# peleiden/rl-rubiks

Hardware: NVIDIA B200
Metric: cube_moves_per_sec (higher is better)
Workload: dtype u8

## Files before the change

### include/rubiks_b200.h

```cpp
#ifndef RUBIKS_B200_H
#define RUBIKS_B200_H

#include <stdint.h>

#ifdef __cplusplus
extern "C" {
#endif

#define RB_OK              0
#define RB_ERR_BAD_ARG     1
#define RB_ERR_CUDA        2
#define RB_ERR_RANGE       3
#define RB_ERR_CAPACITY    4

#define RB_REP_2024        0
#define RB_REP_686         1

#define RB_REWARD_PAPER      0
#define RB_REWARD_LAPANFIX   1
#define RB_REWARD_SCHULTZFIX 2
#define RB_REWARD_REWARD0    3

typedef void* rb_stream_t;

int         rb_version(void);
const char* rb_last_error(void);
int64_t     rb_launch_count(void);

int rb_get_delta_maps(int8_t* delta);
int rb_get_lut2024(uint8_t* lut);
int rb_get_perm686(uint8_t* perm);
int rb_get_macro_table(uint32_t* rows);
int rb_get_macro3_table(uint32_t* rows);
int rb_get_macro3_dedup(uint32_t* elems, uint32_t* remap);
int rb_get_stickers686(uint8_t* corner_home, uint8_t* corner_dst, uint8_t* edge_home, uint8_t* edge_dst);
int rb_get_solved(int rep, int8_t* state);

int rb_multi_rotate(int rep, const int8_t* states, const uint8_t* faces, const uint8_t* dirs,
                    int8_t* out, int64_t n, rb_stream_t stream);
int rb_multi_is_solved(int rep, const int8_t* states, uint8_t* flags, int64_t n, rb_stream_t stream);
int rb_as_oh(int rep, const int8_t* states, float* oh, int64_t n, rb_stream_t stream);
int rb_as_correct_686(const float* oh, float* out, int64_t n, rb_stream_t stream);
int rb_expand12(int rep, const int8_t* states, int8_t* children, float* children_oh,
                uint8_t* solved, int64_t n, rb_stream_t stream);
int rb_check_range(int rep, const int8_t* states, int64_t n_states, const uint8_t* faces,
                   const uint8_t* dirs, int64_t n_actions, int32_t* scratch_dev, rb_stream_t stream);

int rb_scramble(int rep, const uint8_t* actions, int64_t stride_cube, int64_t stride_move,
                const int8_t* start, int8_t* out, int64_t n, int32_t depth, rb_stream_t stream);
int rb_sequence_scramble(int rep, const uint8_t* faces, const uint8_t* dirs, int32_t games, int32_t depth,
                         int32_t with_solved, int8_t* states, float* oh, uint8_t* solved, rb_stream_t stream);

int rb_scramble_seeded(int rep, uint64_t seed, uint64_t first_cube, const int8_t* start, int8_t* out, int64_t n,
                       int32_t depth, rb_stream_t stream);
int rb_seeded_actions(uint64_t seed, uint64_t first_cube, uint8_t* actions, int64_t n, int32_t depth, rb_stream_t stream);
int rb_unpack_actions(const uint8_t* packed, uint8_t* actions, int64_t n, int32_t depth, rb_stream_t stream);

int rb_as686(const int8_t* states2024, int8_t* states686, int64_t n, rb_stream_t stream);
int rb_as2024(const int8_t* states686, int8_t* states2024, uint8_t* ok, int64_t n, rb_stream_t stream);

int rb_adi_generate(int rep, const uint8_t* faces, const uint8_t* dirs, int32_t games, int32_t depth,
                    int32_t with_solved, int8_t* states, float* oh_states, int8_t* children,
                    float* children_oh, uint8_t* solved_states, uint8_t* solved_children, rb_stream_t stream);

int rb_as_oh_bf16(int rep, const int8_t* states, uint16_t* oh, int64_t n, rb_stream_t stream);
int rb_expand12_bf16(int rep, const int8_t* states, int8_t* children, uint16_t* children_oh,
                     uint8_t* solved, int64_t n, rb_stream_t stream);
int rb_sequence_scramble_bf16(int rep, const uint8_t* faces, const uint8_t* dirs, int32_t games, int32_t depth,
                              int32_t with_solved, int8_t* states, uint16_t* oh, uint8_t* solved, rb_stream_t stream);
int rb_adi_generate_bf16(int rep, const uint8_t* faces, const uint8_t* dirs, int32_t games, int32_t depth,
                         int32_t with_solved, int8_t* states, uint16_t* oh_states, int8_t* children,
                         uint16_t* children_oh, uint8_t* solved_states, uint8_t* solved_children, rb_stream_t stream);
int rb_adi_targets(const float* values, const uint8_t* solved_children, const uint8_t* solved_states,
                   int64_t n, int32_t depth, int32_t reward_method, int64_t* policy, float* value,
                   rb_stream_t stream);
int rb_adi_targets_weights(const float* values, const uint8_t* solved_children, const uint8_t* solved_states,
                           int32_t games, int32_t depth, int32_t reward_method, double alpha, double ws,
                           int64_t* policy, float* value, float* loss_weights, rb_stream_t stream);
double rb_adi_weight_sum(int32_t games, int32_t depth);
int rb_adi_loss_weights(float* out, int32_t games, int32_t depth, double alpha, double ws, rb_stream_t stream);

int64_t rb_hashset_bytes(int64_t capacity);
int rb_hashset_clear(void* table, int64_t capacity, rb_stream_t stream);
int rb_hashset_rehash(void* src, int64_t src_capacity, void* dst, int64_t dst_capacity, rb_stream_t stream);
int64_t rb_hashset_scratch_bytes(int64_t n);
int rb_hashset_insert_unique(int rep, void* table, int64_t capacity, const int8_t* states, int64_t n,
                             int32_t* count_dev, uint8_t* seen, uint8_t* first, int32_t* index,
// ... 52 lines not shown
```

### rl_rubiks_b200/_native.py

```python
from __future__ import annotations

import ctypes as C
import os

_HERE = os.path.dirname(os.path.abspath(__file__))
LIB_PATH = os.environ.get("RB_LIB_PATH") or os.path.join(_HERE, "librubiks_b200.so")

RB_OK, RB_ERR_BAD_ARG, RB_ERR_CUDA, RB_ERR_RANGE, RB_ERR_CAPACITY = 0, 1, 2, 3, 4
REP_2024, REP_686 = 0, 1
REWARD_METHODS = {"paper": 0, "lapanfix": 1, "schultzfix": 2, "reward0": 3}

if not os.path.exists(LIB_PATH):
	raise ImportError(
		f"{LIB_PATH} is missing: build it with `python -c 'import __graft_entry__ as g; g.build()'` "
		"(nvcc, sm_100a).  rl_rubiks_b200 has no CPU fallback.")

lib = C.CDLL(LIB_PATH)

_p, _i32, _i64, _f64 = C.c_void_p, C.c_int32, C.c_int64, C.c_double

SIGNATURES = {
	"rb_version": (C.c_int, []),
	"rb_last_error": (C.c_char_p, []),
	"rb_launch_count": (_i64, []),
	"rb_get_delta_maps": (C.c_int, [_p]),
	"rb_get_lut2024": (C.c_int, [_p]),
	"rb_get_perm686": (C.c_int, [_p]),
	"rb_get_macro_table": (C.c_int, [_p]),
	"rb_get_macro3_table": (C.c_int, [_p]),
	"rb_get_macro3_dedup": (C.c_int, [_p, _p]),
	"rb_get_stickers686": (C.c_int, [_p, _p, _p, _p]),
	"rb_get_solved": (C.c_int, [C.c_int, _p]),
	"rb_multi_rotate": (C.c_int, [C.c_int, _p, _p, _p, _p, _i64, _p]),
	"rb_multi_is_solved": (C.c_int, [C.c_int, _p, _p, _i64, _p]),
	"rb_as_oh": (C.c_int, [C.c_int, _p, _p, _i64, _p]),
	"rb_as_correct_686": (C.c_int, [_p, _p, _i64, _p]),
	"rb_expand12": (C.c_int, [C.c_int, _p, _p, _p, _p, _i64, _p]),
	"rb_check_range": (C.c_int, [C.c_int, _p, _i64, _p, _p, _i64, _p, _p]),
	"rb_scramble": (C.c_int, [C.c_int, _p, _i64, _i64, _p, _p, _i64, _i32, _p]),
	"rb_sequence_scramble": (C.c_int, [C.c_int, _p, _p, _i32, _i32, _i32, _p, _p, _p, _p]),
	"rb_adi_generate": (C.c_int, [C.c_int, _p, _p, _i32, _i32, _i32, _p, _p, _p, _p, _p, _p, _p]),
	"rb_as_oh_bf16": (C.c_int, [C.c_int, _p, _p, _i64, _p]),
	"rb_expand12_bf16": (C.c_int, [C.c_int, _p, _p, _p, _p, _i64, _p]),
	"rb_sequence_scramble_bf16": (C.c_int, [C.c_int, _p, _p, _i32, _i32, _i32, _p, _p, _p, _p]),
	"rb_adi_generate_bf16": (C.c_int, [C.c_int, _p, _p, _i32, _i32, _i32, _p, _p, _p, _p, _p, _p, _p]),
	"rb_adi_targets": (C.c_int, [_p, _p, _p, _i64, _i32, _i32, _p, _p, _p]),
	"rb_adi_targets_weights": (C.c_int, [_p, _p, _p, _i32, _i32, _i32, _f64, _f64, _p, _p, _p, _p]),
	"rb_adi_weight_sum": (_f64, [_i32, _i32]),
	"rb_adi_loss_weights": (C.c_int, [_p, _i32, _i32, _f64, _f64, _p]),
	"rb_hashset_bytes": (_i64, [_i64]),
	"rb_hashset_clear": (C.c_int, [_p, _i64, _p]),
	"rb_hashset_rehash": (C.c_int, [_p, _i64, _p, _i64, _p]),
	"rb_hashset_scratch_bytes": (_i64, [_i64]),
	"rb_hashset_insert_unique": (C.c_int, [C.c_int, _p, _i64, _p, _i64, _p, _p, _p, _p, _p, _p]),
	"rb_hashset_lookup": (C.c_int, [C.c_int, _p, _i64, _p, _i64, _p, _p, _p]),
	"rb_frontier_expand": (C.c_int, [C.c_int, _p, _i64, _p, _i64, _p, _p, _p, _p, _p, _p, _p, _p, _p, _p, _p]),
	"rb_frontier_expand_dev": (C.c_int, [C.c_int, _p, _i64, _p, _i64, _p, _p, _p, _p, _p, _p, _p, _p, _p]),
	"rb_frontier_expand_chain": (C.c_int, [C.c_int, _p, _i64, _p, _p, _i64, _i32, _p, _p, _p, _p]),
	"rb_frontier_scratch_bytes": (_i64, [C.c_int, _i64]),
	"rb_astar_scratch_bytes": (_i64, [_i32, _i32]),
	"rb_astar_init": (C.c_int, [_p, _p, _p]),
	"rb_astar_expand": (C.c_int, [_p, _i64, _p, _p, _p, _p, _p, _p]),
	"rb_astar_commit": (C.c_int, [_p, _p, _f64, _p, _p, _p, _p]),
	"rb_as686": (C.c_int, [_p, _p, _i64, _p]),
	"rb_as2024": (C.c_int, [_p, _p, _p, _i64, _p]),
	"rb_scramble_seeded": (C.c_int, [C.c_int, C.c_uint64, C.c_uint64, _p, _p, _i64, _i32, _p]),
	"rb_seeded_actions": (C.c_int, [C.c_uint64, C.c_uint64, _p, _i64, _i32, _p]),
	"rb_unpack_actions": (C.c_int, [_p, _p, _i64, _i32, _p]),
	"rbh_scramble": (C.c_int, [C.c_int, _p, _p, _i64, _i32]),
	"rbh_scramble_packed": (C.c_int, [C.c_int, _p, _p, _i64, _i32]),
	"rbh_scramble_seeded": (C.c_int, [C.c_int, C.c_uint64, C.c_uint64, _p, _i64, _i32]),
	"rbh_multi_rotate": (C.c_int, [C.c_int, _p, _p, _p, _p, _i64]),
	"rbh_host_alloc": (_p, [_i64, C.c_int]),
	"rbh_host_free": (C.c_int, [_p, _i64]),
	"rbh_release": (C.c_int, []),
}

for _name, (_res, _args) in SIGNATURES.items():
	_fn = getattr(lib, _name)
	_fn.restype, _fn.argtypes = _res, _args


class AStarView(C.Structure):
# ... 32 lines not shown
```

### rl_rubiks_b200/csrc/rb_scramble_macro.cuh

```cuda
#pragma once
#include "rb_common.cuh"
#include "rb_tables.cuh"
#include <cuda.h>
#include <array>
#include <map>

namespace rbs {

constexpr int kA = 13;
constexpr int kRows = kA * kA;
constexpr int kRowWords = 5;
constexpr int kDevRows = 256;
constexpr int kP1Bytes = kDevRows * 8 * 16;
constexpr int kP2Bytes = kDevRows * 32 * 4;
constexpr int kTableBytes = kP1Bytes + kP2Bytes;
constexpr int kMaxThreads = 1024;
constexpr int kSmemBudget = 227 * 1024;
constexpr int kReduceEvery = 10;

__device__ __align__(16) uint32_t g_macro[kRows * kRowWords + 3];
__device__ __align__(16) uint32_t g_macro3[12 * 12 * 12 * kRowWords + 3];
__device__ __align__(16) uint32_t g_macro_tail_inv[13 * 13 * kRowWords + 3];

struct Elem {
	uint8_t csrc[8], ctw[8], esrc[12], efl[12];
};

static inline bool neg_chirality(int pos) { return pos == 0 || pos == 2 || pos == 5 || pos == 7; }
static inline int twist_of(int pos, int ori) { return neg_chirality(pos) ? (3 - ori) % 3 : ori; }

static bool single(const rbt::Tables& t, int a, Elem& e) {
	for (int q = 0; q < 8; ++q) { e.csrc[q] = (uint8_t)q; e.ctw[q] = 0; }
	for (int q = 0; q < 12; ++q) { e.esrc[q] = (uint8_t)q; e.efl[q] = 0; }
	if (a == 12) return true;
	for (int p = 0; p < 8; ++p) {
		int delta = -1, dst = -1;
		for (int o = 0; o < 3; ++o) {
			const int v = t.lut[a][0][3 * p + o], p2 = v / 3, o2 = v % 3;
			const int d = (twist_of(p2, o2) - twist_of(p, o) + 3) % 3;
			if (o == 0) { delta = d; dst = p2; }
			else if (d != delta || p2 != dst) return false;
		}
		e.csrc[dst] = (uint8_t)p;
		e.ctw[dst] = (uint8_t)delta;
	}
	for (int p = 0; p < 12; ++p) {
		const int v0 = t.lut[a][1][2 * p], v1 = t.lut[a][1][2 * p + 1];
		if (v0 / 2 != v1 / 2 || ((v0 % 2) ^ 0) != ((v1 % 2) ^ 1)) return false;
		e.esrc[v0 / 2] = (uint8_t)p;
		e.efl[v0 / 2] = (uint8_t)(v0 % 2);
	}
	return true;
}

static void compose(const Elem& x, const Elem& y, Elem& r) {
	for (int q = 0; q < 8; ++q) {
		r.csrc[q] = x.csrc[y.csrc[q]];
		r.ctw[q] = (uint8_t)((x.ctw[y.csrc[q]] + y.ctw[q]) % 3);
	}
	for (int q = 0; q < 12; ++q) {
		r.esrc[q] = x.esrc[y.esrc[q]];
		r.efl[q] = (uint8_t)(x.efl[y.esrc[q]] ^ y.efl[q]);
	}
}

static void encode(const Elem& e, uint32_t* row) {
	uint32_t sc = 0, tf = 0;
	for (int q = 0; q < 8; ++q) sc |= (uint32_t)e.csrc[q] << (4 * q);
	for (int i = 0; i < 4; ++i) tf |= ((uint32_t)e.ctw[i] | ((uint32_t)e.ctw[4 + i] << 2)) << (8 * i);
	row[0] = sc;
	for (int d = 0; d < 3; ++d) {
		uint32_t sa = 0, sb = 0;
		for (int i = 0; i < 4; ++i) {
			const int s = e.esrc[4 * d + i];
			sa |= (uint32_t)(s < 8 ? s : 0) << (4 * i);
			sb |= (uint32_t)(s < 8 ? i : 4 + (s - 8)) << (4 * i);
			tf |= (uint32_t)e.efl[4 * d + i] << (8 * i + 4 + d);
		}
		row[1 + d] = sa | (sb << 16);
	}
	row[4] = tf;
}

constexpr int kRows3 = 12 * 12 * 12;

constexpr int kElems3 = 1080;
constexpr int kRepDedup = 8;
constexpr int kSingle3 = 15 + 12 * 15 + 144 * 15 + 1;
constexpr int kRemap3 = kSingle3 + 16;
constexpr int kElemBytes3 = kElems3 * kRepDedup * 16;
constexpr int kImageBytes3 = kElemBytes3 + kRemap3 * 8;
__device__ __align__(16) uint32_t g_macro3_image[kImageBytes3 / 4];

struct Host {
	uint32_t rows[kRows * kRowWords + 3];
	uint32_t rows3[kRows3 * kRowWords + 3];
	uint32_t rows3_inv[kRows3 * kRowWords + 3];
	uint32_t rows_inv[kRows * kRowWords + 3];
	uint32_t elems3[kElems3 * 4];
	uint32_t remap3[kRemap3 * 2];
	uint32_t image3[kImageBytes3 / 4];
	bool ok;
};

static const Host& host() {
	static Host h;
	static std::once_flag once;
	std::call_once(once, [] {
		memset(&h, 0, sizeof(h));
		const rbt::Tables& t = rbt::host();
		Elem s[kA];
		h.ok = true;
		for (int a = 0; a < kA; ++a) h.ok = single(t, a, s[a]) && h.ok;
		for (int a1 = 0; a1 < kA; ++a1)
			for (int a0 = 0; a0 < kA; ++a0) {
				Elem x;
				compose(s[a0], s[a1], x);
				encode(x, h.rows + (a0 + kA * a1) * kRowWords);
				if (a0 < 12 && a1 < 12)
					for (int a2 = 0; a2 < 12; ++a2) {
						Elem y;
						compose(x, s[a2], y);
						encode(y, h.rows3 + (a0 + 12 * a1 + 144 * a2) * kRowWords);
					}
			}
		auto inv = [](int a) { return a < 12 ? a ^ 1 : a; };
		for (int i = 0; i < kRows3; ++i) {
			const int j = inv(i % 12) + 12 * inv(i / 12 % 12) + 144 * inv(i / 144);
			memcpy(h.rows3_inv + i * kRowWords, h.rows3 + j * kRowWords, sizeof(uint32_t) * kRowWords);
		}
		for (int i = 0; i < kRows; ++i) {
			const int j = inv(i % kA) + kA * inv(i / kA);
			memcpy(h.rows_inv + i * kRowWords, h.rows + j * kRowWords, sizeof(uint32_t) * kRowWords);
		}

		std::map<std::array<uint32_t, 4>, uint32_t> elem;
		auto element_of = [&](const uint32_t* r) {
			const std::array<uint32_t, 4> key{r[0], r[1], r[2], r[3]};
			auto it = elem.find(key);
			if (it != elem.end()) return it->second;
			const uint32_t e = (uint32_t)elem.size();
			if (e < (uint32_t)kElems3) memcpy(h.elems3 + 4 * e, r, 16);
			elem.emplace(key, e);
			return e;
		};
		for (int i = 0; i < kRows3; ++i) {
			const uint32_t* r = h.rows3_inv + i * kRowWords;
			h.remap3[2 * i] = r[4];
			h.remap3[2 * i + 1] = element_of(r);
		}
		for (int a = 0; a < 12; ++a) {
			uint32_t r[kRowWords];
			encode(s[a ^ 1], r);
			h.remap3[2 * (kSingle3 + a)] = r[4];
			h.remap3[2 * (kSingle3 + a) + 1] = element_of(r);
		}
		h.ok = h.ok && elem.size() == (size_t)kElems3;
		auto same = [&](int i, const uint32_t* r) {
			const uint32_t e = h.remap3[2 * i + 1];
			return e < (uint32_t)kElems3 && memcmp(h.elems3 + 4 * e, r, 16) == 0 && h.remap3[2 * i] == r[4];
		};
		for (int i = 0; i < kRows3; ++i) h.ok = h.ok && same(i, h.rows3_inv + i * kRowWords);
		for (int a = 0; a < 12; ++a) h.ok = h.ok && same(kSingle3 + a, h.rows_inv + (a + kA * 12) * kRowWords);
		for (int e = 0; e < kElems3; ++e)
			for (int c = 0; c < kRepDedup; ++c) memcpy(h.image3 + (e * kRepDedup + c) * 4, h.elems3 + 4 * e, 16);
		memcpy(h.image3 + kElemBytes3 / 4, h.remap3, sizeof(h.remap3));
	});
	return h;
}

__device__ __forceinline__ uint32_t smem_u32(const void* p) { return (uint32_t)__cvta_generic_to_shared(p); }

__device__ __forceinline__ void mbar_init(uint64_t* bar, uint32_t count) {
	asm volatile("mbarrier.init.shared::cta.b64 [%0], %1;" ::"r"(smem_u32(bar)), "r"(count) : "memory");
}
__device__ __forceinline__ void mbar_expect_tx(uint64_t* bar, uint32_t bytes) {
	asm volatile("mbarrier.arrive.expect_tx.shared::cta.b64 _, [%0], %1;" ::"r"(smem_u32(bar)), "r"(bytes) : "memory");
}
__device__ __forceinline__ void mbar_wait(uint64_t* bar, uint32_t parity) {
	asm volatile(
		"{\n\t"
		".reg .pred p;\n\t"
		"WAIT_%=:\n\t"
		"mbarrier.try_wait.parity.shared::cta.b64 p, [%0], %1;\n\t"
		"@p bra DONE_%=;\n\t"
		"bra WAIT_%=;\n\t"
		"DONE_%=:\n\t"
		"}" ::"r"(smem_u32(bar)), "r"(parity) : "memory");
}
__device__ __forceinline__ void bulk_g2s(void* dst_smem, const void* src_gmem, uint32_t bytes, uint64_t* bar) {
	asm volatile("cp.async.bulk.shared::cluster.global.mbarrier::complete_tx::bytes [%0], [%1], %2, [%3];" ::"r"(smem_u32(dst_smem)),
	             "l"(src_gmem), "r"(bytes), "r"(smem_u32(bar))
	             : "memory");
}

__device__ __forceinline__ void tma_2d_g2s(void* dst_smem, const CUtensorMap* map, int32_t x, int32_t y, uint64_t* bar) {
	asm volatile("cp.async.bulk.tensor.2d.shared::cluster.global.tile.mbarrier::complete_tx::bytes [%0], [%1, {%2, %3}], [%4];" ::"r"(smem_u32(dst_smem)),
	             "l"(map), "r"(x), "r"(y), "r"(smem_u32(bar))
	             : "memory");
}

struct Slots {
	uint32_t C0, C1, E0, E1, E2;
};

__device__ __forceinline__ uint32_t prmt(uint32_t a, uint32_t b, uint32_t sel) {
	uint32_t r;
	asm("prmt.b32 %0, %1, %2, %3;" : "=r"(r) : "r"(a), "r"(b), "r"(sel));
	return r;
}
template <int k>
__device__ __forceinline__ uint32_t shr_fma(uint32_t x) {
	uint32_t r;
	asm("mul.hi.u32 %0, %1, %2;" : "=r"(r) : "r"(x), "r"(1u << (32 - k)));
	return r;
}

__device__ __forceinline__ uint32_t shr16(uint32_t x) {
	uint32_t r;
// ... 120 lines not shown
				for (; m < depth; m += 2) {
					const uint32_t a0 = row[m], a1 = m + 1 < depth ? row[m + 1] : 12u;
					apply_at(table, row_offset((a0 & 15u) + 13u * (a1 & 15u), lane_off), d2, s);
				}
			}
			store_state(row, s);
		}
		__syncwarp();
		{
			uint8_t* dst = reinterpret_cast<uint8_t*>(out) + chunk * 32 * out_pitch;
			if (kWordAligned && (reinterpret_cast<uintptr_t>(out) & 3u) == 0) {
				for (int i = lane; i < cnt * 5; i += 32) {
					const int c = i / 5, k = i - 5 * c;
					*reinterpret_cast<uint32_t*>(dst + c * out_pitch + 4 * k) = *reinterpret_cast<const uint32_t*>(buf + c * depth + 4 * k);
				}
			} else {
				for (int i = lane; i < cnt * 20; i += 32) {
					const int c = i / 20, k = i - 20 * c;
					dst[c * out_pitch + k] = buf[c * depth + k];
				}
			}
		}
		asm volatile("fence.proxy.async.shared::cta;" ::: "memory");
		__syncwarp();
		if (lane == 0 && chunk + stride < n_chunks) issue(chunk + stride);
	}
}

constexpr int kRep1 = 4;
constexpr int kIdxMax3 = 15 + 12 * 15 + 144 * 15;
constexpr int kP1Bytes3 = kRows3 * kRep1 * 16;
constexpr int kP2Rows3 = 2368;
constexpr int kP2Bytes3 = kP2Rows3 * 4;
constexpr int kTailBytes = kDevRows * 32;
constexpr int kTableBytes3 = kP1Bytes3 + kP2Bytes3 + kTailBytes;
constexpr int kMinSmem3 = (kIdxMax3 + 1) * kRep1 * 16 + 128;

__device__ __forceinline__ uint32_t mad_u32(uint32_t a, uint32_t b, uint32_t c) {
	uint32_t o;
	asm("mad.lo.u32 %0, %1, %2, %3;" : "=r"(o) : "r"(a), "r"(b), "r"(c));
	return o;
}

__device__ __forceinline__ uint4 lds128(uint32_t a) {
	uint4 v;
	asm("ld.shared.v4.u32 {%0, %1, %2, %3}, [%4];" : "=r"(v.x), "=r"(v.y), "=r"(v.z), "=r"(v.w) : "r"(a));
	return v;
}
__device__ __forceinline__ uint32_t lds32(uint32_t a) {
	uint32_t v;
	asm("ld.shared.u32 %0, [%1];" : "=r"(v) : "r"(a));
	return v;
}
__device__ __forceinline__ uint2 lds64(uint32_t a) {
	uint2 v;
	asm("ld.shared.v2.u32 {%0, %1}, [%2];" : "=r"(v.x), "=r"(v.y) : "r"(a));
	return v;
}

__device__ __forceinline__ void stage_table3(uint8_t* table) {
	for (int i = threadIdx.x; i < kP2Rows3 * kRep1; i += blockDim.x) {
		const int row = i / kRep1, c = i % kRep1;
		if (row < kRows3) {
			const uint32_t* r = g_macro3 + row * kRowWords;
			*reinterpret_cast<uint4*>(table + (row * kRep1 + c) * 16) = make_uint4(r[0], r[1], r[2], r[3]);
			if (c == 0) *reinterpret_cast<uint32_t*>(table + kP1Bytes3 + row * 4) = r[4];
		} else if (c == 0) {
			*reinterpret_cast<uint32_t*>(table + kP1Bytes3 + row * 4) = 0u;
		}
	}
	uint8_t* tail = table + kP1Bytes3 + kP2Bytes3;
	for (int i = threadIdx.x; i < kDevRows; i += blockDim.x) {
		const uint32_t* r = g_macro_tail_inv + (i < kRows ? i : kRows - 1) * kRowWords;
		*reinterpret_cast<uint4*>(tail + i * 32) = make_uint4(r[0], r[1], r[2], r[3]);
		*reinterpret_cast<uint32_t*>(tail + i * 32 + 16) = r[4];
	}
}

__device__ __forceinline__ void fold(Slots& s) { s.C0 = fold_twists(s.C0); s.C1 = fold_twists(s.C1); }

template <bool kDedup>
struct Rows3 {
	uint32_t off1, off2, tail, p1_stride, p2_stride;

	__device__ __forceinline__ Rows3(const uint8_t* table, uint32_t lane, uint32_t p1, uint32_t p2)
		: off1(smem_u32(table) + (lane & ((kDedup ? kRepDedup : kRep1) - 1)) * 16u),
		  off2(smem_u32(table) + (kDedup ? (uint32_t)kElemBytes3 : (uint32_t)kP1Bytes3)),
		  tail(smem_u32(table + kP1Bytes3 + kP2Bytes3)), p1_stride(p1), p2_stride(p2) {}

	__device__ __forceinline__ void apply3(Slots& s, uint32_t r) const {
		if (kDedup) {
			const uint2 e = lds64(mad_u32(r, p2_stride, off2));
			apply_row(lds128(mad_u32(e.y, p1_stride, off1)), e.x, s);
		} else {
			const uint32_t o1 = mad_u32(r, 16u * kRep1, off1), o2 = mad_u32(r, p2_stride, off2);
			apply_row(lds128(o1), lds32(o2), s);
		}
	}
	__device__ __forceinline__ void apply1(Slots& s, uint32_t a) const { apply3(s, (uint32_t)kSingle3 + a); }
	__device__ __forceinline__ void apply_tail(Slots& s, uint32_t idx2) const {
		const uint32_t r = tail + idx2 * 32u;
		apply_row(lds128(r), lds32(r + 16u), s);
	}
	__device__ __forceinline__ void apply_words(Slots& s, uint32_t w0, uint32_t w1, uint32_t w2) const {
		w0 &= 0x0f0f0f0fu; w1 &= 0x0f0f0f0fu; w2 &= 0x0f0f0f0fu;
		apply3(s, __dp4a(w2, 0x010C9000u, 0u));
		apply3(s, __dp4a(w2, 0x00000001u, __dp4a(w1, 0x0C900000u, 0u)));
		apply3(s, __dp4a(w1, 0x0000010Cu, __dp4a(w0, 0x90000000u, 0u)));
		apply3(s, __dp4a(w0, 0x00010C90u, 0u));
	}
	__device__ __forceinline__ void rem8(Slots& s, uint32_t wa, uint32_t wb) const {
		wa &= 0x0f0f0f0fu; wb &= 0x0f0f0f0fu;
		apply3(s, __dp4a(wb, 0x010C9000u, 0u));
		apply3(s, __dp4a(wb, 0x00000001u, __dp4a(wa, 0x0C900000u, 0u)));
		if (kDedup) { apply1(s, (wa >> 8) & 0xffu); apply1(s, wa & 0xffu); }
		else apply_tail(s, __dp4a(wa, 0x0000010Du, 0u));
	}
	__device__ __forceinline__ void rem4(Slots& s, uint32_t wa) const {
		wa &= 0x0f0f0f0fu;
		apply3(s, __dp4a(wa, 0x010C9000u, 0u));
		if (kDedup) apply1(s, wa & 0xffu);
		else apply_tail(s, (wa & 0xffu) + 13u * 12u);
	}
	__device__ __forceinline__ void group24(Slots& s, uint32_t w0, uint32_t w1, uint32_t w2, uint32_t w3, uint32_t w4, uint32_t w5) const {
		apply_words(s, w3, w4, w5); apply_words(s, w0, w1, w2);
		fold(s);
	}
};

template <bool kWords, bool kDedup, class WordAt, class InvAt>
__device__ __forceinline__ void walk3(const Rows3<kDedup>& t, Slots& s, int depth, WordAt word_at, InvAt inv_at) {
	const int M = depth - depth % 24;
	int pos = depth;
	if (pos > M) {
		if (kWords) {
			if (pos - 12 >= M) { t.apply_words(s, word_at(pos - 12), word_at(pos - 8), word_at(pos - 4)); pos -= 12; }
			if (pos - 8 >= M) t.rem8(s, word_at(pos - 8), word_at(pos - 4));
			else if (pos - 4 >= M) t.rem4(s, word_at(pos - 4));
		} else {
			for (; pos - 3 >= M; pos -= 3) t.apply3(s, inv_at(pos - 1) + 12u * inv_at(pos - 2) + 144u * inv_at(pos - 3));
			if (kDedup) {
				for (; pos > M; --pos) t.apply1(s, inv_at(pos - 1));
			} else if (pos > M) {
				t.apply_tail(s, inv_at(pos - 1) + 13u * (pos - 2 >= M ? inv_at(pos - 2) : 12u));
			}
		}
// ... 8 lines not shown
template <int kCubes>
__device__ __forceinline__ void store_results(int8_t* out, int64_t first, int out_pitch, int cnt, uint32_t tid, const uint32_t (&w)[5]) {
	uint8_t* dst = reinterpret_cast<uint8_t*>(out) + first * out_pitch;
	if (out_pitch == 20 && (reinterpret_cast<uintptr_t>(out) & 3u) == 0) {
#pragma unroll
		for (int t = 0; t < 5; ++t) {
			const int j = (int)tid + kCubes * t;
			if (j < cnt * 5) reinterpret_cast<uint32_t*>(dst)[j] = w[t];
		}
	} else if ((reinterpret_cast<uintptr_t>(out) & 3u) == 0 && (out_pitch & 3) == 0) {
#pragma unroll
		for (int t = 0; t < 5; ++t) {
			const int j = (int)tid + kCubes * t, c = j / 5, k = j - 5 * c;
			if (j < cnt * 5) *reinterpret_cast<uint32_t*>(dst + c * out_pitch + 4 * k) = w[t];
		}
	} else {
#pragma unroll
		for (int t = 0; t < 5; ++t) {
			const int j = (int)tid + kCubes * t, c = j / 5, k = j - 5 * c;
			if (j < cnt * 5)
				for (int q = 0; q < 4; ++q) dst[c * out_pitch + 4 * k + q] = (uint8_t)(w[t] >> (8 * q));
		}
	}
}

__device__ __forceinline__ uint32_t mod3_bytes_folded(uint32_t c) {
	uint32_t t = (c & 0x03030303u) + ((c >> 2) & 0x03030303u);
	t = (t & 0x03030303u) + ((t >> 2) & 0x01010101u);
	const uint32_t x = t & (t >> 1) & 0x01010101u;
	return t ^ (x * 3u);
}

__device__ __forceinline__ void cubie_major(const Slots& s, uint32_t (&w)[5]) {
#pragma unroll
	for (int h = 0; h < 2; ++h) {
		const uint32_t c = h ? s.C1 : s.C0;
		const uint32_t t = mod3_bytes_folded(c);
		const uint32_t sw = ((t << 1) & 0x02020202u) | ((t >> 1) & 0x01010101u);
		const uint32_t p = (c >> 5) & 0x07070707u;
		const uint32_t neg = (((p ^ (p >> 2)) & 0x01010101u) ^ 0x01010101u) * 255u;
		w[h] = p * 3u + ((t & neg) | (sw & ~neg));
	}
#pragma unroll
	for (int d = 0; d < 3; ++d) {
		const uint32_t e = d == 0 ? s.E0 : (d == 1 ? s.E1 : s.E2);
		const uint32_t f = ((e >> 4) ^ (e >> 5) ^ (e >> 6)) & 0x01010101u;
		w[2 + d] = ((e & 0x0f0f0f0fu) << 1) + f;
	}
}

template <int kMode, bool kDedup>
__global__ void __launch_bounds__(kMaxThreads, 1)
k_scramble_macro3(const uint8_t* __restrict__ actions, int8_t* __restrict__ out, int64_t n, int depth, int out_pitch,
                  uint32_t p1_stride, uint32_t p2_stride, uint32_t n_work) {
	constexpr bool kWordAligned = kMode >= 1;
	extern __shared__ __align__(128) uint8_t smem[];
	uint8_t* table = smem;
	uint64_t* tbar = reinterpret_cast<uint64_t*>(smem + kImageBytes3);
	uint64_t* bars = reinterpret_cast<uint64_t*>(kDedup ? smem + kImageBytes3 + 16 : smem + kTableBytes3);
	const uint32_t lane = threadIdx.x & 31, wib = threadIdx.x >> 5, n_warps = n_work;
	const int chunk_bytes = 32 * depth;
	constexpr bool a16 = kMode >= 2, pad16 = kMode == 3;
	const int pitch = depth + (pad16 ? 16 : 0);
	uint8_t* buf = reinterpret_cast<uint8_t*>(bars) + kMaxThreads / 32 * 8 + (size_t)wib * (32 * pitch);
	uint64_t* bar = &bars[wib];
	const Rows3<kDedup> t(table, lane, p1_stride, p2_stride);

	const int64_t n_chunks = (n + 31) / 32;
	const int64_t stride = (int64_t)gridDim.x * n_warps;
	int64_t chunk = (int64_t)blockIdx.x * n_warps + wib;

	auto issue = [&](int64_t c) {
		if (c >= n_chunks) return;
		const int cnt = (int)min((int64_t)32, n - c * 32);
		if (pad16) {
			if (lane == 0) mbar_expect_tx(bar, (uint32_t)(cnt * depth));
			__syncwarp();
			if ((int)lane < cnt) bulk_g2s(buf + lane * pitch, actions + c * chunk_bytes + (int64_t)lane * depth, (uint32_t)depth, bar);
		} else if (lane == 0) {
			const uint32_t bulk = (uint32_t)(cnt * depth) & ~15u;
			if (bulk) {
				mbar_expect_tx(bar, bulk);
				bulk_g2s(buf, actions + c * chunk_bytes, bulk, bar);
			}
		}
	};
	if (kDedup && threadIdx.x == 0) mbar_init(tbar, 1);
	if (lane == 0) mbar_init(bar, 1);
	asm volatile("fence.mbarrier_init.release.cluster;" ::: "memory");
	__syncwarp();
	if (kDedup && threadIdx.x == 0) {
		mbar_expect_tx(tbar, (uint32_t)kImageBytes3);
		bulk_g2s(table, g_macro3_image, (uint32_t)kImageBytes3, tbar);
	}
	if (wib < n_work) issue(chunk);
	if (!kDedup) stage_table3(table);
	__syncthreads();
	if (wib >= n_work) return;
	if (kDedup) mbar_wait(tbar, 0);

	uint32_t parity = 0;
	for (; chunk < n_chunks; chunk += stride) {
		const int cnt = (int)min((int64_t)32, n - chunk * 32);
		const int bytes = cnt * depth, bulk = bytes & ~15;
		if (bulk < bytes) {
			if ((int)lane < bytes - bulk) buf[bulk + lane] = actions[chunk * chunk_bytes + bulk + lane];
			__syncwarp();
		}
		if (bulk) { mbar_wait(bar, parity); parity ^= 1u; }

		uint32_t res[5] = {0u, 0u, 0u, 0u, 0u};
		if ((int)lane < cnt) {
			uint8_t* row = buf + lane * pitch;
			Slots s{0x60402000u, 0xe0c0a080u, 0x03020100u, 0x07060504u, 0x0b0a0908u};
			const uint32_t* arow = reinterpret_cast<const uint32_t*>(buf + ((lane * depth) & ~3));
			const uint32_t ashift = ((lane * depth) & 3) * 8;
			auto word_at = [&](int m) -> uint32_t {
				if (kWordAligned) return *reinterpret_cast<const uint32_t*>(row + m);
				return __funnelshift_r(arow[m >> 2], arow[(m >> 2) + 1], ashift);
// ... 197 lines not shown
}

static int box_height(int depth) {
	if (depth <= 256) return depth;
	for (int k = (depth + 255) / 256; k <= 16; ++k)
		if (depth % k == 0 && (depth / k) % 4 == 0) return depth / k;
	return 0;
}

static bool can_transposed(const uint8_t* actions, int64_t n, int depth) {
	return depth >= 20 && n % 16 == 0 && n < (int64_t(1) << 31) && (reinterpret_cast<uintptr_t>(actions) & 15u) == 0 && box_height(depth) > 0 &&
	       encode_tiled_fn() != nullptr;
}

static int quads_for(int64_t n, int depth) {
	if (depth < 20) return 0;
	int64_t q = (kSmemBudget - 16 - kFixedSmem3) / ((int64_t)kSpan * depth);
	if (q > kMaxThreads / 128) q = kMaxThreads / 128;
	if (q < 2) return 0;
	const int64_t spread = ((n + kSpan - 1) / kSpan + RB_NUM_SMS - 1) / RB_NUM_SMS;
	if (q > spread) q = spread;
	return (int)q;
}

static int launch_mm(const uint8_t* actions, int8_t* out, int64_t n, int depth, cudaStream_t st, int out_pitch) {
	int rc = ensure_device();
	if (rc != RB_OK) return rc;
	const int Q = quads_for(n, depth), bh = box_height(depth);
	if (Q <= 0 || bh <= 0) return rb_fail(RB_ERR_BAD_ARG, "move-major fast path does not apply%s%s");
	CUtensorMap tmap;
	const cuuint64_t gdim[2] = {(cuuint64_t)n, (cuuint64_t)depth}, gstride[1] = {(cuuint64_t)n};
	const cuuint32_t box[2] = {(cuuint32_t)kSpan, (cuuint32_t)bh}, estride[2] = {1u, 1u};
	const CUresult cr = encode_tiled_fn()(&tmap, CU_TENSOR_MAP_DATA_TYPE_UINT8, 2, const_cast<uint8_t*>(actions), gdim, gstride, box, estride,
	                                      CU_TENSOR_MAP_INTERLEAVE_NONE, CU_TENSOR_MAP_SWIZZLE_NONE, CU_TENSOR_MAP_L2_PROMOTION_L2_128B,
	                                      CU_TENSOR_MAP_FLOAT_OOB_FILL_NONE);
	if (cr != CUDA_SUCCESS) return rb_fail(RB_ERR_CUDA, "cuTensorMapEncodeTiled failed for the move-major action array%s%s");
	const int64_t spans = (n + kSpan - 1) / kSpan, ctas = (spans + Q - 1) / Q;
	const int grid = (int)(ctas < RB_NUM_SMS ? ctas : RB_NUM_SMS);
	size_t smem = (size_t)kFixedSmem3 + (size_t)Q * kSpan * depth + 16;
	if (smem < (size_t)kMinSmem3) smem = kMinSmem3;
	if (depth % 4 == 0) k_scramble_mm<true><<<grid, kStageThreads, smem, st>>>(tmap, out, n, depth, out_pitch, 4u, (uint32_t)Q, bh);
	else k_scramble_mm<false><<<grid, kStageThreads, smem, st>>>(tmap, out, n, depth, out_pitch, 4u, (uint32_t)Q, bh);
	RB_LAUNCHED("scramble_mm_2024");
	return RB_OK;
}

template <bool kDedup>
static int launch3(const uint8_t* actions, int8_t* out, int64_t n, int depth, cudaStream_t st, int out_pitch, int W3) {
	const int64_t ctas = ((n + 31) / 32 + W3 - 1) / W3;
	const int grid = (int)(ctas < RB_NUM_SMS ? ctas : RB_NUM_SMS);
	const int threads = kDedup || W3 * 32 >= kStageThreads ? W3 * 32 : kStageThreads;
	size_t smem = (size_t)(kDedup ? kFixedSmemDedup : kFixedSmem3) + (size_t)W3 * 32 * pitch3(depth) + 16;
	if (smem < (size_t)kMinSmem3) smem = kMinSmem3;
	const uint32_t p1 = kDedup ? kRepDedup * 16u : 0u, p2 = kDedup ? 8u : 4u, nw = (uint32_t)W3;
	if (depth % 4 != 0) k_scramble_macro3<0, kDedup><<<grid, threads, smem, st>>>(actions, out, n, depth, out_pitch, p1, p2, nw);
	else if (depth % 128 == 0) k_scramble_macro3<3, kDedup><<<grid, threads, smem, st>>>(actions, out, n, depth, out_pitch, p1, p2, nw);
	else if (depth % 16 == 0) k_scramble_macro3<2, kDedup><<<grid, threads, smem, st>>>(actions, out, n, depth, out_pitch, p1, p2, nw);
	else k_scramble_macro3<1, kDedup><<<grid, threads, smem, st>>>(actions, out, n, depth, out_pitch, p1, p2, nw);
	RB_LAUNCHED("scramble_macro3_2024");
	return RB_OK;
}

static int launch(const uint8_t* actions, int8_t* out, int64_t n, int depth, cudaStream_t st, int out_pitch) {
	int rc = ensure_device();
	if (rc != RB_OK) return rc;
	const bool dedup = smem_warps3(depth, true) >= 12;
	const int W3 = warps_for3(n, depth, dedup);
	if (W3 > 0) return dedup ? launch3<true>(actions, out, n, depth, st, out_pitch, W3) : launch3<false>(actions, out, n, depth, st, out_pitch, W3);
	const int W = warps_for(n, depth);
	const int64_t ctas = ((n + 31) / 32 + W - 1) / W;
	const int grid = (int)(ctas < RB_NUM_SMS ? ctas : RB_NUM_SMS);
	const size_t smem = (size_t)kFixedSmem + (size_t)W * 32 * depth;
	if (depth % 4 == 0) k_scramble_macro<true><<<grid, W * 32, smem, st>>>(actions, out, n, depth, out_pitch);
	else k_scramble_macro<false><<<grid, W * 32, smem, st>>>(actions, out, n, depth, out_pitch);
	RB_LAUNCHED("scramble_macro_2024");
	return RB_OK;
}

}
```

### rl_rubiks_b200/csrc/rubiks_b200.cu

```cuda
#include <sys/mman.h>
#include "rb_common.cuh"
#include "rb_tables.cuh"
#include "rb_cube2024.cuh"
#include "rb_scramble_macro.cuh"
#include "rb_scramble_seeded.cuh"
#include "rb_cube686.cuh"
#include "rb_adi.cuh"
#include "rb_frontier.cuh"
#include "rb_astar.cuh"
#include "rb_host.cuh"

#define RB_INIT()                                   \
	do {                                            \
		int rc_ = rbt::ensure_device();             \
		if (rc_ != RB_OK) return rc_;               \
	} while (0)

static inline bool aligned(const void* p, uintptr_t a) { return (reinterpret_cast<uintptr_t>(p) & (a - 1)) == 0; }
static inline cudaStream_t S(rb_stream_t s) { return reinterpret_cast<cudaStream_t>(s); }
static inline bool rep_ok(int rep) { return rep == RB_REP_2024 || rep == RB_REP_686; }

extern "C" {

int rb_version(void) { return 100; }
const char* rb_last_error(void) { return g_rb_err; }
int64_t rb_launch_count(void) { return g_rb_launches.load(); }

int rb_get_delta_maps(int8_t* delta) {
	RB_REQUIRE(delta, "null output");
	memcpy(delta, rbt::host().delta, sizeof(rbt::host().delta));
	return RB_OK;
}
int rb_get_lut2024(uint8_t* lut) {
	RB_REQUIRE(lut, "null output");
	memcpy(lut, rbt::host().lut, sizeof(rbt::host().lut));
	return RB_OK;
}
int rb_get_perm686(uint8_t* perm) {
	RB_REQUIRE(perm, "null output");
	memcpy(perm, rbt::host().perm686, sizeof(rbt::host().perm686));
	return RB_OK;
}
int rb_get_macro_table(uint32_t* rows) {
	RB_REQUIRE(rows, "null output");
	const rbs::Host& h = rbs::host();
	if (!h.ok) return rb_fail(RB_ERR_BAD_ARG, "macro-move tables: a host check failed (twist additivity or the deduplicated 3-move table)%s%s");
	memcpy(rows, h.rows, sizeof(uint32_t) * rbs::kRows * rbs::kRowWords);
	return RB_OK;
}
int rb_get_macro3_table(uint32_t* rows) {
	RB_REQUIRE(rows, "null output");
	const rbs::Host& h = rbs::host();
	if (!h.ok) return rb_fail(RB_ERR_BAD_ARG, "macro-move tables: a host check failed (twist additivity or the deduplicated 3-move table)%s%s");
	memcpy(rows, h.rows3, sizeof(uint32_t) * rbs::kRows3 * rbs::kRowWords);
	return RB_OK;
}
int rb_get_macro3_dedup(uint32_t* elems, uint32_t* remap) {
	RB_REQUIRE(elems && remap, "null output");
	const rbs::Host& h = rbs::host();
	if (!h.ok) return rb_fail(RB_ERR_BAD_ARG, "macro-move tables: a host check failed (twist additivity or the deduplicated 3-move table)%s%s");
	memcpy(elems, h.elems3, sizeof(h.elems3));
	memcpy(remap, h.remap3, sizeof(h.remap3));
	return RB_OK;
}
int rb_get_stickers686(uint8_t* corner_home, uint8_t* corner_dst, uint8_t* edge_home, uint8_t* edge_dst) {
	RB_REQUIRE(corner_home && corner_dst && edge_home && edge_dst, "null output");
	const rbt::Tables& t = rbt::host();
	if (!t.stickers_ok) return rb_fail(RB_ERR_BAD_ARG, "sticker tables: the 20x24 and 6x8x6 move tables disagree%s%s");
	memcpy(corner_home, t.corner_home, sizeof(t.corner_home));
	memcpy(corner_dst, t.corner_dst, sizeof(t.corner_dst));
	memcpy(edge_home, t.edge_home, sizeof(t.edge_home));
	memcpy(edge_dst, t.edge_dst, sizeof(t.edge_dst));
	return RB_OK;
}
int rb_get_solved(int rep, int8_t* state) {
	RB_REQUIRE(state && rep_ok(rep), "bad argument");
	if (rep == RB_REP_2024) memcpy(state, rbt::host().solved2024, 20);
	else memcpy(state, rbt::host().solved686, 288);
	return RB_OK;
}

int rb_multi_rotate(int rep, const int8_t* states, const uint8_t* faces, const uint8_t* dirs, int8_t* out,
                    int64_t n, rb_stream_t stream) {
	RB_REQUIRE(rep_ok(rep) && n >= 0, "bad rep or size");
	if (n == 0) return RB_OK;
	RB_REQUIRE(states && faces && out, "null pointer");
	RB_INIT();
	if (rep == RB_REP_2024) {
		if (aligned(states, 4) && aligned(out, 4))
			rb2024::k_multi_rotate<<<rb_grid(n, 256, 5), rb2024::kThreads, 0, S(stream)>>>(states, faces, dirs, out, n);
		else
			rb2024::k_multi_rotate_any<<<rb_grid(n, rb2024::kTile, 2), rb2024::kThreads, 0, S(stream)>>>(states, faces, dirs, out, n);
		RB_LAUNCHED("multi_rotate_2024");
	} else {
		RB_REQUIRE(aligned(states, 4) && aligned(out, 4), "6x8x6 states must be 4-byte aligned");
		rb686::k_multi_rotate<<<rb_grid(n, rb686::kMrStates * rb686::kWarps, 5), rb686::kThreads, 0, S(stream)>>>(states, faces, dirs, out, n);
		RB_LAUNCHED("multi_rotate_686");
	}
	return RB_OK;
}

int rb_multi_is_solved(int rep, const int8_t* states, uint8_t* flags, int64_t n, rb_stream_t stream) {
	RB_REQUIRE(rep_ok(rep) && n >= 0, "bad rep or size");
	if (n == 0) return RB_OK;
	RB_REQUIRE(states && flags, "null pointer");
	RB_INIT();
	if (rep == RB_REP_2024) {
		if (aligned(states, 4))
			rb2024::k_is_solved<<<rb_grid(n, 256, 8), rb2024::kThreads, 0, S(stream)>>>(states, flags, n);
		else
			rb2024::k_is_solved_any<<<rb_grid(n, rb2024::kTile, 2), rb2024::kThreads, 0, S(stream)>>>(states, flags, n);
		RB_LAUNCHED("is_solved_2024");
	} else {
		RB_REQUIRE(aligned(states, 4), "6x8x6 states must be 4-byte aligned");
		rb686::k_is_solved<<<rb_grid(n, 4 * rb686::kWarps, 8), rb686::kThreads, 0, S(stream)>>>(states, flags, n);
// ... 721 lines not shown
```

Measured before the change: 2211 billion.

## Replace dedup 3-move remap pair with perfect-hashed single-word lookup

The deduplicated 3-move table now stores one 32-bit word per macro row instead of an (effect, element index) pair. The permutation element is found through a multiplicative perfect hash into 1136 slots, built on the host with an augmenting-path assignment that uses the free twist and bit-7 encodings. This swaps the 64-bit shared load in the inner apply3 for a 32-bit load plus a mul.hi, which shrinks the remap region, at the cost of a larger element image (1136 slots instead of the unique element count). Host checks confirm that twist overflow stays bounded even with the redundant encoded bits.

```diff
diff --git a/include/rubiks_b200.h b/include/rubiks_b200.h
--- a/include/rubiks_b200.h
+++ b/include/rubiks_b200.h
@@ -33,6 +33,7 @@
 int rb_get_macro_table(uint32_t* rows);
 int rb_get_macro3_table(uint32_t* rows);
 int rb_get_macro3_dedup(uint32_t* elems, uint32_t* remap);
+int rb_get_macro3_image(uint32_t* image, uint32_t* hash_mul);
 int rb_get_stickers686(uint8_t* corner_home, uint8_t* corner_dst, uint8_t* edge_home, uint8_t* edge_dst);
 int rb_get_solved(int rep, int8_t* state);
 
diff --git a/rl_rubiks_b200/_native.py b/rl_rubiks_b200/_native.py
--- a/rl_rubiks_b200/_native.py
+++ b/rl_rubiks_b200/_native.py
@@ -29,6 +29,7 @@
 	"rb_get_macro_table": (C.c_int, [_p]),
 	"rb_get_macro3_table": (C.c_int, [_p]),
 	"rb_get_macro3_dedup": (C.c_int, [_p, _p]),
+	"rb_get_macro3_image": (C.c_int, [_p, _p]),
 	"rb_get_stickers686": (C.c_int, [_p, _p, _p, _p]),
 	"rb_get_solved": (C.c_int, [C.c_int, _p]),
 	"rb_multi_rotate": (C.c_int, [C.c_int, _p, _p, _p, _p, _i64, _p]),
diff --git a/rl_rubiks_b200/csrc/rb_scramble_macro.cuh b/rl_rubiks_b200/csrc/rb_scramble_macro.cuh
--- a/rl_rubiks_b200/csrc/rb_scramble_macro.cuh
+++ b/rl_rubiks_b200/csrc/rb_scramble_macro.cuh
@@ -2,8 +2,11 @@
 #include "rb_common.cuh"
 #include "rb_tables.cuh"
 #include <cuda.h>
+#include <algorithm>
 #include <array>
+#include <functional>
 #include <map>
+#include <vector>
 
 namespace rbs {
 
@@ -88,9 +91,20 @@
 constexpr int kRepDedup = 8;
 constexpr int kSingle3 = 15 + 12 * 15 + 144 * 15 + 1;
 constexpr int kRemap3 = kSingle3 + 16;
-constexpr int kElemBytes3 = kElems3 * kRepDedup * 16;
-constexpr int kImageBytes3 = kElemBytes3 + kRemap3 * 8;
+constexpr int kSlots3 = 1136;
+constexpr int kThree3[2] = {0, 2};
+constexpr int kElemBytes3 = kSlots3 * kRepDedup * 16;
+constexpr int kImageBytes3 = kElemBytes3 + kRemap3 * 4;
 __device__ __align__(16) uint32_t g_macro3_image[kImageBytes3 / 4];
+
+static inline uint32_t slot3(uint32_t w, uint32_t mul) { return (uint32_t)(((uint64_t)(w * mul) * (uint32_t)kSlots3) >> 32); }
+static inline int twist_shift(int q) { return 8 * (q & 3) + 2 * (q >> 2); }
+static inline uint32_t tf_effect(uint32_t w) {
+	w &= 0x7f7f7f7fu;
+	for (int q = 0; q < 8; ++q)
+		if (((w >> twist_shift(q)) & 3u) == 3u) w &= ~(3u << twist_shift(q));
+	return w;
+}
 
 struct Host {
 	uint32_t rows[kRows * kRowWords + 3];
@@ -99,6 +113,9 @@
 	uint32_t rows_inv[kRows * kRowWords + 3];
 	uint32_t elems3[kElems3 * 4];
 	uint32_t remap3[kRemap3 * 2];
+	uint32_t words3[kRemap3];
+	uint16_t slot_elem3[kSlots3];
+	uint32_t hash_mul3;
 	uint32_t image3[kImageBytes3 / 4];
 	bool ok;
 };
@@ -162,9 +179,86 @@
 		};
 		for (int i = 0; i < kRows3; ++i) h.ok = h.ok && same(i, h.rows3_inv + i * kRowWords);
 		for (int a = 0; a < 12; ++a) h.ok = h.ok && same(kSingle3 + a, h.rows_inv + (a + kA * 12) * kRowWords);
-		for (int e = 0; e < kElems3; ++e)
-			for (int c = 0; c < kRepDedup; ++c) memcpy(h.image3 + (e * kRepDedup + c) * 4, h.elems3 + 4 * e, 16);
-		memcpy(h.image3 + kElemBytes3 / 4, h.remap3, sizeof(h.remap3));
+		if (!h.ok) return;
+
+		uint32_t tf[kElems3];
+		for (int i = 0; i < kRows3; ++i) tf[h.remap3[2 * i + 1]] = h.remap3[2 * i];
+		auto src = [&](uint32_t e, int q) { return (int)((h.elems3[4 * e] >> (4 * q)) & 15u); };
+		auto in_three = [](int q) { return q == kThree3[0] || q == kThree3[1]; };
+		std::vector<std::vector<uint32_t>> cand(kElems3);
+		for (int e = 0; e < kElems3; ++e) {
+			std::vector<uint32_t> extra{0u};
+			for (int d : kThree3)
+				if (((tf[e] >> twist_shift(d)) & 3u) == 0 && !in_three(src(e, d)))
+					for (size_t k = 0, n = extra.size(); k < n; ++k) extra.push_back(extra[k] | 3u << twist_shift(d));
+			for (uint32_t x : extra)
+				for (uint32_t key = 0; key < 16; ++key) {
+					uint32_t k7 = 0;
+					for (int i = 0; i < 4; ++i) k7 |= ((key >> i) & 1u) << (8 * i + 7);
+					cand[e].push_back(tf[e] | x | k7);
+				}
+		}
+		std::vector<int> order(kElems3), owner(kSlots3), stamp(kSlots3, 0);
+		std::vector<uint32_t> key(kElems3);
+		for (int e = 0; e < kElems3; ++e) order[e] = e;
+		std::stable_sort(order.begin(), order.end(), [&](int a, int b) { return cand[a].size() < cand[b].size(); });
+		int visit = 0;
+		uint32_t mul = 0;
+		std::function<bool(int)> place = [&](int e) {
+			for (uint32_t w : cand[e]) {
+				const uint32_t s = slot3(w, mul);
+				if (stamp[s] == visit) continue;
+				stamp[s] = visit;
+				if (owner[s] == -1 || (owner[s] >= 0 && place(owner[s]))) {
+					owner[s] = e;
+					key[e] = w;
+					return true;
+				}
+			}
+			return false;
+		};
+		bool placed = false;
+		for (int tries = 0; !placed && tries < 64; ++tries) {
+			mul = tries ? (mul + 0x6A09E668u) | 1u : 0x9E3779B1u;
+			std::fill(owner.begin(), owner.end(), -1);
+			owner[0] = -2;
+			placed = true;
+			for (int e : order) {
+				++visit;
+				if (!place(e)) { placed = false; break; }
+			}
+		}
+		h.ok = placed;
+		if (!h.ok) return;
+		h.hash_mul3 = mul;
+		for (int s = 0; s < kSlots3; ++s) h.slot_elem3[s] = (uint16_t)(owner[s] >= 0 ? owner[s] : 0);
+		for (int i = 0; i < kRemap3; ++i) {
+			const bool valid = i < kRows3 || (i >= kSingle3 && i < kSingle3 + 12);
+			h.words3[i] = valid ? key[h.remap3[2 * i + 1]] : 0u;
+		}
+		for (int i = 0; i < kRemap3; ++i) {
+			const uint32_t w = h.words3[i];
+			h.ok = h.ok && h.slot_elem3[slot3(w, mul)] == h.remap3[2 * i + 1] && tf_effect(w) == h.remap3[2 * i];
+		}
+		auto worst_gain = [&](int rows) {
+			int f[8] = {0, 0, 0, 0, 0, 0, 0, 0};
+			for (int k = 0; k < rows; ++k) {
+				int g[8] = {0, 0, 0, 0, 0, 0, 0, 0};
+				for (int i = 0; i < kRemap3; ++i) {
+					const uint32_t w = h.words3[i], e = h.slot_elem3[slot3(w, mul)];
+					for (int q = 0; q < 8; ++q) {
+						const int p = src(e, q);
+						g[p] = std::max(g[p], (int)((w >> twist_shift(q)) & 3u) + f[q]);
+					}
+				}
+				memcpy(f, g, sizeof(f));
+			}
+			return *std::max_element(f, f + 8);
+		};
+		h.ok = h.ok && 10 + worst_gain(8) <= 31 && worst_gain(9) <= 31;
+		for (int s = 0; s < kSlots3; ++s)
+			for (int c = 0; c < kRepDedup; ++c) memcpy(h.image3 + (s * kRepDedup + c) * 4, h.elems3 + 4 * h.slot_elem3[s], 16);
+		memcpy(h.image3 + kElemBytes3 / 4, h.words3, sizeof(h.words3));
 	});
 	return h;
 }
@@ -391,11 +485,6 @@
 	asm("ld.shared.u32 %0, [%1];" : "=r"(v) : "r"(a));
 	return v;
 }
-__device__ __forceinline__ uint2 lds64(uint32_t a) {
-	uint2 v;
-	asm("ld.shared.v2.u32 {%0, %1}, [%2];" : "=r"(v.x), "=r"(v.y) : "r"(a));
-	return v;
-}
 
 __device__ __forceinline__ void stage_table3(uint8_t* table) {
 	for (int i = threadIdx.x; i < kP2Rows3 * kRep1; i += blockDim.x) {
@@ -420,17 +509,19 @@
 
 template <bool kDedup>
 struct Rows3 {
-	uint32_t off1, off2, tail, p1_stride, p2_stride;
-
-	__device__ __forceinline__ Rows3(const uint8_t* table, uint32_t lane, uint32_t p1, uint32_t p2)
+	uint32_t off1, off2, tail, p1_stride, p2_stride, hash_mul;
+
+	__device__ __forceinline__ Rows3(const uint8_t* table, uint32_t lane, uint32_t p1, uint32_t p2, uint32_t mul = 0u)
 		: off1(smem_u32(table) + (lane & ((kDedup ? kRepDedup : kRep1) - 1)) * 16u),
 		  off2(smem_u32(table) + (kDedup ? (uint32_t)kElemBytes3 : (uint32_t)kP1Bytes3)),
-		  tail(smem_u32(table + kP1Bytes3 + kP2Bytes3)), p1_stride(p1), p2_stride(p2) {}
+		  tail(smem_u32(table + kP1Bytes3 + kP2Bytes3)), p1_stride(p1), p2_stride(p2), hash_mul(mul) {}
 
 	__device__ __forceinline__ void apply3(Slots& s, uint32_t r) const {
 		if (kDedup) {
-			const uint2 e = lds64(mad_u32(r, p2_stride, off2));
-			apply_row(lds128(mad_u32(e.y, p1_stride, off1)), e.x, s);
+			const uint32_t w = lds32(mad_u32(r, p2_stride, off2));
+			uint32_t slot;
+			asm("mul.hi.u32 %0, %1, %2;" : "=r"(slot) : "r"(w * hash_mul), "r"((uint32_t)kSlots3));
+			apply_row(lds128(mad_u32(slot, p1_stride, off1)), w, s);
 		} else {
 			const uint32_t o1 = mad_u32(r, 16u * kRep1, off1), o2 = mad_u32(r, p2_stride, off2);
 			apply_row(lds128(o1), lds32(o2), s);
@@ -545,7 +636,7 @@
 template <int kMode, bool kDedup>
 __global__ void __launch_bounds__(kMaxThreads, 1)
 k_scramble_macro3(const uint8_t* __restrict__ actions, int8_t* __restrict__ out, int64_t n, int depth, int out_pitch,
-                  uint32_t p1_stride, uint32_t p2_stride, uint32_t n_work) {
+                  uint32_t p1_stride, uint32_t p2_stride, uint32_t n_work, uint32_t hash_mul) {
 	constexpr bool kWordAligned = kMode >= 1;
 	extern __shared__ __align__(128) uint8_t smem[];
 	uint8_t* table = smem;
@@ -557,7 +648,7 @@
 	const int pitch = depth + (pad16 ? 16 : 0);
 	uint8_t* buf = reinterpret_cast<uint8_t*>(bars) + kMaxThreads / 32 * 8 + (size_t)wib * (32 * pitch);
 	uint64_t* bar = &bars[wib];
-	const Rows3<kDedup> t(table, lane, p1_stride, p2_stride);
+	const Rows3<kDedup> t(table, lane, p1_stride, p2_stride, hash_mul);
 
 	const int64_t n_chunks = (n + 31) / 32;
 	const int64_t stride = (int64_t)gridDim.x * n_warps;
@@ -861,11 +952,11 @@
 	const int threads = kDedup || W3 * 32 >= kStageThreads ? W3 * 32 : kStageThreads;
 	size_t smem = (size_t)(kDedup ? kFixedSmemDedup : kFixedSmem3) + (size_t)W3 * 32 * pitch3(depth) + 16;
 	if (smem < (size_t)kMinSmem3) smem = kMinSmem3;
-	const uint32_t p1 = kDedup ? kRepDedup * 16u : 0u, p2 = kDedup ? 8u : 4u, nw = (uint32_t)W3;
-	if (depth % 4 != 0) k_scramble_macro3<0, kDedup><<<grid, threads, smem, st>>>(actions, out, n, depth, out_pitch, p1, p2, nw);
-	else if (depth % 128 == 0) k_scramble_macro3<3, kDedup><<<grid, threads, smem, st>>>(actions, out, n, depth, out_pitch, p1, p2, nw);
-	else if (depth % 16 == 0) k_scramble_macro3<2, kDedup><<<grid, threads, smem, st>>>(actions, out, n, depth, out_pitch, p1, p2, nw);
-	else k_scramble_macro3<1, kDedup><<<grid, threads, smem, st>>>(actions, out, n, depth, out_pitch, p1, p2, nw);
+	const uint32_t p1 = kDedup ? kRepDedup * 16u : 0u, p2 = 4u, nw = (uint32_t)W3, mul = kDedup ? host().hash_mul3 : 0u;
+	if (depth % 4 != 0) k_scramble_macro3<0, kDedup><<<grid, threads, smem, st>>>(actions, out, n, depth, out_pitch, p1, p2, nw, mul);
+	else if (depth % 128 == 0) k_scramble_macro3<3, kDedup><<<grid, threads, smem, st>>>(actions, out, n, depth, out_pitch, p1, p2, nw, mul);
+	else if (depth % 16 == 0) k_scramble_macro3<2, kDedup><<<grid, threads, smem, st>>>(actions, out, n, depth, out_pitch, p1, p2, nw, mul);
+	else k_scramble_macro3<1, kDedup><<<grid, threads, smem, st>>>(actions, out, n, depth, out_pitch, p1, p2, nw, mul);
 	RB_LAUNCHED("scramble_macro3_2024");
 	return RB_OK;
 }
diff --git a/rl_rubiks_b200/csrc/rubiks_b200.cu b/rl_rubiks_b200/csrc/rubiks_b200.cu
--- a/rl_rubiks_b200/csrc/rubiks_b200.cu
+++ b/rl_rubiks_b200/csrc/rubiks_b200.cu
@@ -61,6 +61,14 @@
 	if (!h.ok) return rb_fail(RB_ERR_BAD_ARG, "macro-move tables: a host check failed (twist additivity or the deduplicated 3-move table)%s%s");
 	memcpy(elems, h.elems3, sizeof(h.elems3));
 	memcpy(remap, h.remap3, sizeof(h.remap3));
+	return RB_OK;
+}
+int rb_get_macro3_image(uint32_t* image, uint32_t* hash_mul) {
+	RB_REQUIRE(image && hash_mul, "null output");
+	const rbs::Host& h = rbs::host();
+	if (!h.ok) return rb_fail(RB_ERR_BAD_ARG, "macro-move tables: a host check failed (twist additivity or the deduplicated 3-move table)%s%s");
+	memcpy(image, h.image3, sizeof(h.image3));
+	*hash_mul = h.hash_mul3;
 	return RB_OK;
 }
 int rb_get_stickers686(uint8_t* corner_home, uint8_t* corner_dst, uint8_t* edge_home, uint8_t* edge_dst) {
```

Result: slower. 2163 billion, median of 6 (-2.2%).
